# bcgsc/NanoSim

Measured on AMD Instinct MI355X. Metric: simulated reads/sec (genome mode, mean 8 kb), higher is better.
Workload: dtype u8

## Files before the change

### nanosim_amd/csrc/nanosim_amd.hip

```cpp
#include <hip/hip_runtime.h>
#include <hipcub/hipcub.hpp>
#include <stdio.h>
#include <stdlib.h>
#include <string.h>
#include <algorithm>
#include <chrono>
#include <atomic>
#include <condition_variable>
#include <functional>
#include <mutex>
#include <thread>
#include <type_traits>
#include <string>
#include <vector>

#include "ns_device.h"
#include "ns_materialise.h"
#include "ns_chain.h"
#include "ns_hp.h"
#include "ns_ir.h"
#include "ns_io.h"
#include "ns_pack.h"
#include "ns_cs_hist.h"
#include "ns_qual_hist.h"
// ... 965 lines not shown
    rd.rec_off = uni64(A.rec_off[r]);
    rd.piece_off = uni(rd.piece_off); rd.n_pieces = (uint16_t)uni(rd.n_pieces);
    rd.reversed = (uint8_t)uni(rd.reversed); rd.head = uni(rd.head); rd.tail = uni(rd.tail); rd.seq_len = uni(rd.seq_len);
    rd.attempts = uni(rd.attempts);
    key = read_key(A, r);
    key.r_lo = uni(key.r_lo); key.r_hi = uni(key.r_hi);
    ro.seq = A.records + rd.rec_off + uni(A.name_len[r]) + 2;
    ro.qual = fastq ? ro.seq + rd.seq_len + 3 : nullptr;
    ro.seq_len = rd.seq_len; ro.reversed = rd.reversed != 0; ro.uracil = A.prm.uracil != 0;
    return true;
}

#ifndef NS_MATQ_WAVES
#define NS_MATQ_WAVES 4
#endif
#ifndef NS_MATQ_MINW
#define NS_MATQ_MINW 6
#endif
__device__ __forceinline__ uint64_t hp_ev_slot(uint32_t hp_shift, uint32_t hp_pad, uint64_t pos, uint32_t piece) { return (pos >> hp_shift) + (uint64_t)hp_pad * piece; }
__device__ __forceinline__ uint64_t hp_ev_slot(const GenArgs &A, uint64_t pos, uint32_t piece) { return hp_ev_slot(A.hp_shift, A.hp_pad, pos, piece); }

#ifndef NS_TILE_CHUNKS_FINAL
#define NS_TILE_CHUNKS_FINAL 4u
#endif
#ifndef NS_MAT_WAVES_FINAL
#define NS_MAT_WAVES_FINAL 6
#endif
struct MatArgs { GenArgs A; SlowQueue sq; const uint32_t *order; uint32_t dbg; };
typedef const __attribute__((address_space(4))) MatArgs *MatArgsPtr;
__device__ __forceinline__ MatArgsPtr mat_args_now() {
    MatArgsPtr p = (MatArgsPtr)__builtin_amdgcn_kernarg_segment_ptr();
    asm volatile("" : "+s"(p));
    return p;
}
struct MatCold {
    uint32_t gp, pi;
    __device__ __forceinline__ void push(uint32_t lane, uint32_t m0, uint32_t m1) const {
        const uint32_t *order = mat_args_now()->order;
        const uint32_t r = order ? uni(order[blockIdx.x]) : blockIdx.x;
        const MatArgsPtr K = mat_args_now();
        SlowQueue sq; sq.items = K->sq.items; sq.count = K->sq.count; sq.cap = K->sq.cap;
        slow_queue_push(sq, lane, SlowTile{r, pi, m0, m1});
    }
    __device__ __forceinline__ uint64_t chrom_len() const {
        const MatArgsPtr K = mat_args_now();
        const ns_piece *pieces = K->A.pieces;
        const uint64_t *off = K->A.ref.chrom_off;
        const uint32_t chrom = uni(pieces[gp].chrom);
        return uni64(off[chrom + 1]) - uni64(off[chrom]);
    }
};

template <bool FASTQ, int MODE, uint32_t TC, bool URACIL>
__device__ __forceinline__ uint32_t materialise_pieces(const GenArgs &A, TileLds<TC> &T, const ReadOut &ro, const ns_key &key, const ns_read &rd,
                                                       uint64_t r, uint32_t q, uint32_t lane, uint32_t dbg) {
    constexpr bool CLSOUT = FASTQ && MODE != MAT_HP_SCRATCH;
    const uint32_t a = rd.attempts;
    uint32_t *cls = nullptr;
    if constexpr (CLSOUT) cls = A.cls + cls_word0(rd.rec_off, r, cls_per_read(A.prm));
    uint64_t q_in = MODE == MAT_HP_FINAL ? uni64(A.scr_off[r]) : 0;
    for (uint32_t pi = 0; pi < rd.n_pieces; ++pi) {
        PieceCtx pc;
        const uint32_t gp = rd.piece_off + pi;
        if constexpr (MODE == MAT_HP_FINAL) {
            const MatArgsPtr K = mat_args_now();
            const ns_piece *pieces = K->A.pieces;
            const uint32_t *hp_pord = K->A.hp_pord, *hp_nev = K->A.hp_nev, *hp_len = K->A.hp_len;
            const ns_piece p = pieces[gp];
            const uint64_t eo = hp_ev_slot(K->A.hp_shift, K->A.hp_pad, q_in, uni(hp_pord[r]) + pi);
            pc.kind = uni(p.kind);
            pc.ev = K->A.hp_ev + eo; pc.wd = K->A.hp_wd + eo; pc.n_ev = pc.kind ? 0u : uni(hp_nev[gp]);
            pc.ref_len = uni(p.out_len); pc.out_len = pc.kind ? pc.ref_len : uni(hp_len[gp]);
            pc.chrom_base = (uint64_t)((uintptr_t)K->A.scr - (uintptr_t)K->A.ref.bases) + q_in; pc.chrom_len = ~0ull; pc.pos = 0;
            pc.sid = pc.kind ? NS_GAP_SEG + (pi >> 1) : (pi >> 1);
            q_in += pc.ref_len;
        } else pc = load_piece_uniform(A.events, A.ref, A.pieces[gp], pi);
        uint32_t *const pcls = CLSOUT ? cls + (q >> 4) + 2u * pi : nullptr;
        if (ro.reversed) materialise_piece<FASTQ, MODE, TC, true, URACIL>(A.ref, T, PieceOut<true>(ro, q), key, a, pc, lane, dbg, MatCold{gp, pi}, pcls);
        else materialise_piece<FASTQ, MODE, TC, false, URACIL>(A.ref, T, PieceOut<false>(ro, q), key, a, pc, lane, dbg, MatCold{gp, pi}, pcls);
        q += pc.out_len;
    }
    return q;
}

template <bool FASTQ, int MODE, bool URACIL>
__global__ void __launch_bounds__(64, MODE == MAT_HP_FINAL ? NS_MAT_WAVES_FINAL : NS_MAT_WAVES)
k_materialise(MatArgs K) {
    static_assert(std::is_trivially_copyable<MatArgs>::value && offsetof(MatArgs, A) == 0, "MatArgs is read back from the kernel-argument segment as it was passed");
    constexpr uint32_t TC = MODE == MAT_HP_FINAL ? NS_TILE_CHUNKS_FINAL : NS_TILE_CHUNKS;
    __shared__ TileLds<TC> T;
    const GenArgs &A = K.A;
    const uint32_t lane = threadIdx.x;
    const uint64_t slot = blockIdx.x;
    if (slot >= A.prm.n_reads) return;
    const uint64_t r = K.order ? (uint64_t)uni(K.order[slot]) : slot;
    ns_read rd; ns_key key; ReadOut ro;
    if (!load_read_uniform(A, r, false, rd, key, ro)) return;
    tile_lds_init(T, lane);
    if constexpr (MODE == MAT_HP_SCRATCH) {
        static_assert(MODE != MAT_HP_SCRATCH || !URACIL, "the scratch pass of -k writes T");
        ro.seq = A.scr + uni64(A.scr_off[r]); ro.qual = nullptr; ro.reversed = false; ro.uracil = false;
        materialise_pieces<FASTQ, MODE, TC, false>(A, T, ro, key, rd, r, 0u, lane, K.dbg);
    } else {
        ro.uracil = URACIL;
#ifdef NS_ABLATE
        if (!(K.dbg & 8))
#endif
        emit_head_tail(ro, key, rd.attempts, rd.head, rd.tail, lane);
        const uint32_t q = materialise_pieces<FASTQ, MODE, TC, URACIL>(A, T, ro, key, rd, r, rd.head, lane, K.dbg);
        if (A.polya) {
            const uint32_t pl = uni(A.polya[r]);
            if (pl) emit_polya(ro, q, pl, lane);
        }
    }
}

template <bool HPF>
__global__ void __launch_bounds__(64 * NS_MATQ_WAVES, NS_MATQ_MINW) k_qualities(GenArgs A, const uint32_t *order) {
    __shared__ __align__(16) uint16_t qlut[NS_QLUT_SLOTS * 1024u];
    qual_lut_load(qlut, A.m, threadIdx.x, 64 * NS_MATQ_WAVES);
    __syncthreads();
    const uint32_t lane = threadIdx.x & 63u;
    const uint64_t slot = (uint64_t)blockIdx.x * NS_MATQ_WAVES + (threadIdx.x >> 6);
    if (slot >= A.prm.n_reads) return;
    const uint64_t r = order ? (uint64_t)uni(order[slot]) : slot;
    ns_read rd; ns_key key; ReadOut ro;
    if (!load_read_uniform(A, r, true, rd, key, ro)) return;
    const uint32_t a = rd.attempts;
    QualState Q; Q.lut = qlut;
    qualities_head_tail(A.m, Q, ro, key, a, rd.head, rd.tail, lane);
    const uint32_t *cls = A.cls + cls_word0(rd.rec_off, r, cls_per_read(A.prm));
    uint32_t q = rd.head;
    for (uint32_t pi = 0; pi < rd.n_pieces; ++pi) {
        const uint32_t gp = rd.piece_off + pi;
        const ns_piece p = A.pieces[gp];
        const uint32_t kind = uni(p.kind);
        const uint32_t out_len = (HPF && !kind) ? uni(A.hp_len[gp]) : uni(p.out_len);
        qualities_piece(A.m, Q, ro, key, a, kind ? NS_GAP_SEG + (pi >> 1) : (pi >> 1), kind, out_len, q, cls + (q >> 4) + 2u * pi, lane);
        q += out_len;
    }
    if (A.polya) {
        const uint32_t pl = uni(A.polya[r]);
        if (pl) emit_polya_quals(A.m, ro, key, a, q, pl, rd.head, rd.tail, lane);
    }
}

#define NS_DENSE_SEG 4096u
__global__ void __launch_bounds__(256) k_dense_plan(GenArgs A, uint32_t *cnt) {
    const uint64_t r = (uint64_t)blockIdx.x * blockDim.x + threadIdx.x;
    if (r > A.prm.n_reads) return;
    uint32_t c = 0;
    if (r < A.prm.n_reads) { const ns_read rd = A.reads[r]; c = rd.flags ? 0u : max(1u, (rd.seq_len + NS_DENSE_SEG - 1u) / NS_DENSE_SEG); }
    cnt[r] = c;
}
__global__ void __launch_bounds__(64) k_materialise_dense(GenArgs A, const uint32_t *__restrict__ seg_off) {
    __shared__ DenseLds S;
    const uint32_t lane = threadIdx.x;
    const uint32_t w = blockIdx.x, n = (uint32_t)A.prm.n_reads;
    if (w >= seg_off[n]) return;
    uint32_t lo = 0, hi = n;
    while (hi - lo > 1) { const uint32_t mid = (lo + hi) >> 1; if (seg_off[mid] <= w) lo = mid; else hi = mid; }
    const uint64_t r = uni(lo);
    const uint32_t seg = uni(w - seg_off[lo]);
    ns_read rd; ns_key key; ReadOut ro;
    if (!load_read_uniform(A, r, false, rd, key, ro)) return;
    const uint32_t a = rd.attempts;
    if (seg == 0) emit_head_tail(ro, key, a, rd.head, rd.tail, lane);
    uint32_t q = rd.head;
    for (uint32_t pi = 0; pi < rd.n_pieces; ++pi) {
        const PieceCtx pc = load_piece_uniform(A.events, A.ref, A.pieces[rd.piece_off + pi], pi);
        const uint64_t s_lo = (uint64_t)seg * NS_DENSE_SEG, s_hi = s_lo + NS_DENSE_SEG, p_lo = q - rd.head, p_hi = p_lo + pc.out_len;
        if (p_hi > s_lo && p_lo < s_hi) {
            const uint32_t m_lo = (uint32_t)(max(s_lo, p_lo) - p_lo), m_hi = (uint32_t)(min(s_hi, p_hi) - p_lo);
            if (A.dbg & 16384u) slow_piece_range(A.m, A.ref, ro, key, a, pc, q, m_lo, m_hi, lane);
            else dense_piece(A.m, A.ref, S, ro, key, a, pc, q, m_lo, m_hi, lane);
        }
        q += pc.out_len;
    }
}

template <bool FASTQ, bool SCRATCH>
__global__ void __launch_bounds__(64) k_materialise_slow(GenArgs A, SlowQueue sq) {
    const uint32_t lane = threadIdx.x;
    const uint32_t n = min(*sq.count, sq.cap);
    for (uint32_t i = blockIdx.x; i < n; i += gridDim.x) {
        const SlowTile t = sq.items[i];
        ns_read rd; ns_key key; ReadOut ro;
        if (!load_read_uniform(A, t.read, FASTQ && !SCRATCH, rd, key, ro)) continue;
        uint32_t q = SCRATCH ? 0u : rd.head;
        if constexpr (SCRATCH) { ro.seq = A.scr + A.scr_off[t.read]; ro.qual = nullptr; ro.reversed = false; ro.uracil = false; }
        for (uint32_t pi = 0; pi < t.piece; ++pi) q += A.pieces[rd.piece_off + pi].out_len;
        const PieceCtx pc = load_piece_uniform(A.events, A.ref, A.pieces[rd.piece_off + t.piece], t.piece);
        slow_piece_range<FASTQ && SCRATCH>(A.m, A.ref, ro, key, rd.attempts, pc, q, t.m0, t.m1, lane);
    }
}

template <bool FASTQ>
__global__ void __launch_bounds__(64) k_materialise_slow_hpf(GenArgs A, SlowQueue sq) {
    const uint32_t lane = threadIdx.x;
    const uint32_t n = min(*sq.count, sq.cap);
    for (uint32_t i = blockIdx.x; i < n; i += gridDim.x) {
        const SlowTile t = sq.items[i];
        ns_read rd; ns_key key; ReadOut ro;
        if (!load_read_uniform(A, t.read, FASTQ, rd, key, ro)) continue;
        uint32_t q = rd.head;
        uint64_t q_in = A.scr_off[t.read];
        for (uint32_t pi = 0; pi < t.piece; ++pi) {
            const uint32_t gp = rd.piece_off + pi;
            const ns_piece p = A.pieces[gp];
            q += p.kind ? p.out_len : A.hp_len[gp];
            q_in += p.out_len;
        }
        const uint32_t gp = rd.piece_off + t.piece;
        const ns_piece p = A.pieces[gp];
        const uint64_t eo = hp_ev_slot(A, q_in, A.hp_pord[t.read] + t.piece);
        const ns_event *ev = A.hp_ev + eo;
        const uint32_t *wd = A.hp_wd + eo;
        const uint32_t n_ev = p.kind ? 0u : A.hp_nev[gp], sid = p.kind ? NS_GAP_SEG + (t.piece >> 1) : (t.piece >> 1);
        const uint8_t *src = A.scr + q_in;
// ... 3059 lines not shown
```

### nanosim_amd/csrc/ns_device.h

```cpp
#pragma once
#include "ns_rng.h"
#include "../../include/nanosim_amd.h"

enum NsStat : uint32_t {
    NS_STAT_OVER,
    NS_STAT_BASES,
    NS_STAT_REF_BASES,
    NS_STAT_EVENTS,
    NS_STAT_MAX_READ,
    NS_STAT_HP_FAILED,
    NS_STAT_NEXT_N,
    NS_STAT_HP_OVER,
    NS_STAT_HP_RANGE,
    NS_STAT_COUNT
};
#define NS_RANGE_SHIFT 40
#define NS_OVER_MASK ((1ull << NS_RANGE_SHIFT) - 1)
#define NS_STATS_WAYS 64u
#define NS_STATS_BYTES ((NS_STAT_COUNT + NS_STAT_COUNT * NS_STATS_WAYS) * sizeof(unsigned long long))
__host__ __device__ inline unsigned long long *ns_stats_way(unsigned long long *stats, uint32_t way) { return stats + NS_STAT_COUNT + NS_STAT_COUNT * way; }

struct ChainTab {
    uint32_t n_words;
    uint32_t trans;
// ... 272 lines not shown
    for (int e = 0; e < 12; ++e) {
        const uint32_t i = (uint32_t)list[e].code & 31u;
        uint32_t k = 0;
        for (; list[e].mem[k]; ++k) {
            const char b = list[e].mem[k];
            p.slot[k] |= (uint64_t)(b == 'A' ? 0 : b == 'T' ? 1 : b == 'C' ? 2 : 3) << (2u * i);
        }
        p.cnt |= (uint64_t)(k - 1u) << (2u * i);
    }
    return p;
}
NS_DEV uint32_t iupac_members(uint32_t c, uint32_t &n) {
    constexpr IupacPack P = iupac_pack();
    const uint32_t sh = 2u * (c & 31u);
    const uint32_t code = (c >> 5) == 2u ? (uint32_t)(P.cnt >> sh) & 3u : 0u;
    n = code + (code != 0u);
    uint32_t mem = 0;
    for (uint32_t k = 0; k < 4u; ++k) mem |= ((0x47435441u >> (8u * ((uint32_t)(P.slot[k] >> sh) & 3u))) & 0xffu) << (8u * k);
    return code ? mem & (0xffffffffu >> (8u * (3u - code))) : 0u;
}
NS_DEV uint8_t normalise_base(uint32_t c) {
    c &= 0x7fu;
    if (c >= 'a' && c <= 'z') c -= 32;
    uint32_t n;
    if (is_acgt(c)) return (uint8_t)c;
    iupac_members(c, n);
    return (uint8_t)((n ? c : (uint32_t)'N') | 0x80u);
}
NS_DEV uint8_t resolve_base(uint32_t c, const ns_key &key, uint32_t seg, uint32_t attempt, uint32_t x) {
    if (!(c & 0x80u)) return (uint8_t)c;
    c &= 0x7fu;
    uint32_t n, mem = iupac_members(c, n);
    if (!n) return (uint8_t)c;
    u32x4 w = ns_draw(key, ST_IUPAC, seg, attempt, x >> 2, 0);
    uint32_t j = (uint32_t)(((uint64_t)ns_word(w, x & 3) * n) >> 32);
    return (uint8_t)(mem >> (8 * j));
}
NS_DEV uint32_t payload_word(const ns_key &key, uint32_t seg, uint32_t attempt, uint32_t j, uint32_t c) {
    if (c == 0) { u32x4 w = ns_draw(key, ST_SUB, seg, attempt, j >> 2, 0); return ns_word(w, j & 3); }
    u32x4 w = ns_draw(key, ST_INS, seg, attempt, j, c >> 2);
    return ns_word(w, c & 3);
}
NS_DEV uint8_t mis_from_digit(uint32_t cur, uint32_t dg) {
    int rc = base_rank(cur);
    uint32_t rk = dg + ((int)dg >= rc ? 1u : 0u);
    if (rc < 0) rk = dg;
    return bases_atcg(rk);
}
NS_DEV uint32_t next_digit3(uint32_t &frac) {
    uint64_t p = (uint64_t)frac * 3u;
    frac = (uint32_t)p;
    return (uint32_t)(p >> 32);
}
__device__ __forceinline__ uint8_t mis_letter(uint32_t cur, const ns_key &key, uint32_t seg, uint32_t attempt, uint32_t j, uint32_t i) {
    uint32_t frac = payload_word(key, seg, attempt, j, i >> 4), dg = 0;
    for (uint32_t t = 0; t <= (i & 15); ++t) dg = next_digit3(frac);
    return mis_from_digit(cur, dg);
}
__device__ __forceinline__ uint8_t ins_letter(const ns_key &key, uint32_t seg, uint32_t attempt, uint32_t j, uint32_t i) {
    return bases_atcg((payload_word(key, seg, attempt, j, i >> 4) >> (2 * (i & 15))) & 3u);
}
__device__ __forceinline__ uint8_t ht_letter(const ns_key &key, uint32_t stream, uint32_t attempt, uint32_t i) {
    u32x4 w = ns_draw(key, stream, 0, attempt, i >> 6, 0);
    return bases_atcg((ns_word(w, (i >> 4) & 3) >> (2 * (i & 15))) & 3u);
}
NS_DEV uint8_t qual_value_lut(const uint32_t *__restrict__ thr, const uint16_t *__restrict__ lut, uint32_t h) {
    const uint32_t e = lut[h >> 6];
    if (!(e & 0x8000u)) return (uint8_t)(((e & 0x7fffu) + (h & 63u)) >> 7);
    uint32_t q = (e >> 7) & 0x7fu;
    while (q < NS_QUAL_LEVELS - 1 && h >= thr[q]) ++q;
    return (uint8_t)q;
}
NS_DEV uint8_t qual_value(const uint32_t *__restrict__ thr, uint32_t h) {
    uint32_t lo = 0, hi = NS_QUAL_LEVELS - 1;
    while (lo < hi) {
        uint32_t mid = (lo + hi) >> 1;
        if (h >= thr[mid]) lo = mid + 1; else hi = mid;
    }
    return (uint8_t)lo;
}
__device__ __forceinline__ uint8_t qual_at(const DevModel &m, int cls, const ns_key &key, uint32_t stream, uint32_t seg,
                                           uint32_t attempt, uint32_t mpos) {
    u32x4 w = ns_draw(key, stream, seg, attempt, mpos >> 3, 0);
    uint32_t h = (ns_word(w, (mpos & 7) >> 1) >> (16 * (mpos & 1))) & 0xffffu;
    return qual_value(m.qual_thr + cls * NS_QUAL_LEVELS, h);
}

NS_DEV uint32_t dec_digits(uint32_t v) {
    return v < 10u ? 1u : v < 100u ? 2u : v < 1000u ? 3u : v < 10000u ? 4u : v < 100000u ? 5u : v < 1000000u ? 6u : v < 10000000u ? 7u :
           v < 100000000u ? 8u : v < 1000000000u ? 9u : 10u;
}
NS_DEV uint8_t *put_dec(uint8_t *p, uint32_t v) {
    const uint32_t n = dec_digits(v);
    for (uint32_t i = 0; i < n; ++i) { const uint32_t q = v / 10u; p[n - 1 - i] = (uint8_t)('0' + (v - 10u * q)); v = q; }
    return p + n;
}
template <class P>
NS_DEV P put_dec_p(P p, uint32_t v) {
    const uint32_t n = dec_digits(v);
    for (uint32_t i = 0; i < n; ++i) { const uint32_t q = v / 10u; p[n - 1 - i] = (uint8_t)('0' + (v - 10u * q)); v = q; }
    return p + n;
}
__device__ __forceinline__ uint32_t dec_digits(uint64_t v) {
    uint32_t n = 1;
    while (v >= 10) { v /= 10; ++n; }
    return n;
// ... 14 lines not shown
```

### nanosim_amd/csrc/ns_materialise.h

```cpp
#pragma once
#include "ns_device.h"

#ifndef NS_TILE_CHUNKS
#define NS_TILE_CHUNKS 2u
#endif
#define T_EV 64u
#define NS_CLS_MIS_BIT 0x08u
#define NS_CLS_INS_BIT 0x20u
#define NS_CLS_STRIP 0xd7d7d7d7u
#define NS_QLUT_SLOTS 5u
__device__ __forceinline__ uint32_t wave_incl_scan(uint32_t v) {
    v += (uint32_t)__builtin_amdgcn_update_dpp(0, (int)v, 0x111, 0xf, 0xf, true);
    v += (uint32_t)__builtin_amdgcn_update_dpp(0, (int)v, 0x112, 0xf, 0xf, true);
    v += (uint32_t)__builtin_amdgcn_update_dpp(0, (int)v, 0x114, 0xf, 0xf, true);
    v += (uint32_t)__builtin_amdgcn_update_dpp(0, (int)v, 0x118, 0xf, 0xf, true);
    v += (uint32_t)__builtin_amdgcn_update_dpp(0, (int)v, 0x142, 0xa, 0xf, false);
    v += (uint32_t)__builtin_amdgcn_update_dpp(0, (int)v, 0x143, 0xc, 0xf, false);
    return v;
}

__device__ __forceinline__ uint32_t wave_incl_max(uint32_t v) {
    v = max(v, (uint32_t)__builtin_amdgcn_update_dpp(0, (int)v, 0x111, 0xf, 0xf, false));
    v = max(v, (uint32_t)__builtin_amdgcn_update_dpp(0, (int)v, 0x112, 0xf, 0xf, false));
    v = max(v, (uint32_t)__builtin_amdgcn_update_dpp(0, (int)v, 0x114, 0xf, 0xf, false));
    v = max(v, (uint32_t)__builtin_amdgcn_update_dpp(0, (int)v, 0x118, 0xf, 0xf, false));
    v = max(v, (uint32_t)__builtin_amdgcn_update_dpp(0, (int)v, 0x142, 0xa, 0xf, false));
    v = max(v, (uint32_t)__builtin_amdgcn_update_dpp(0, (int)v, 0x143, 0xc, 0xf, false));
    return v;
}
__device__ __forceinline__ uint32_t dpp_wave_shl1(uint32_t lane63_value, uint32_t v) {
    return (uint32_t)__builtin_amdgcn_update_dpp((int)lane63_value, (int)v, 0x130, 0xf, 0xf, false);
}

__device__ __forceinline__ uint32_t uni(uint32_t v) { return (uint32_t)__builtin_amdgcn_readfirstlane((int)v); }
__device__ __forceinline__ uint64_t uni64(uint64_t v) { return (uint64_t)uni((uint32_t)v) | (uint64_t)uni((uint32_t)(v >> 32)) << 32; }

__device__ __forceinline__ uint32_t here(uint32_t v) { asm volatile("" : "+s"(v)); return v; }

struct ReadOut {
    uint8_t *seq;
    uint8_t *qual;
    uint32_t seq_len;
    bool reversed;
    bool uracil;
};
__device__ __forceinline__ uint64_t t_to_u8(uint64_t x) {
    const uint64_t t = x ^ 0x5454545454545454ull;
    const uint64_t z = ~(((t & 0x7f7f7f7f7f7f7f7full) + 0x7f7f7f7f7f7f7f7full) | t) & 0x8080808080808080ull;
    return x | (z >> 7);
}

typedef uint32_t ns_v4u_any __attribute__((ext_vector_type(4), aligned(1)));
__device__ __forceinline__ void store16(uint8_t *dst, uint32_t count, uint64_t lo, uint64_t hi) {
    if (count == 16) {
        ns_v4u_any x = {(uint32_t)lo, (uint32_t)(lo >> 32), (uint32_t)hi, (uint32_t)(hi >> 32)};
        __builtin_nontemporal_store(x, reinterpret_cast<ns_v4u_any *>(dst));
    } else {
        if (count & 8u) { __builtin_memcpy(dst, &lo, 8); dst += 8; lo = hi; }
// ... 233 lines not shown
    }
}

__device__ __forceinline__ void wave_sync() {
    __builtin_amdgcn_fence(__ATOMIC_ACQ_REL, "wavefront");
    __builtin_amdgcn_wave_barrier();
}

typedef __attribute__((address_space(3))) volatile uint8_t *LdsBytes;
typedef __attribute__((address_space(3))) volatile uint32_t *LdsWords;
__device__ __forceinline__ void lds_put_bytes(LdsBytes d, uint32_t x0, uint32_t x1, uint32_t x2, uint32_t x3, uint32_t cn) {
    const uint32_t head = min(cn, (0u - (uint32_t)(uintptr_t)d) & 3u);
    if (head > 0) d[0] = (uint8_t)x0;
    if (head > 1) d[1] = (uint8_t)(x0 >> 8);
    if (head > 2) d[2] = (uint8_t)(x0 >> 16);
    const uint32_t sh = 8u * head;
    const uint32_t y0 = __builtin_amdgcn_alignbit(x1, x0, sh), y1 = __builtin_amdgcn_alignbit(x2, x1, sh), y2 = __builtin_amdgcn_alignbit(x3, x2, sh), y3 = x3 >> sh;
    const uint32_t rem = cn - head;
    const LdsWords w = (LdsWords)(d + head);
    if (rem >= 4u) w[0] = y0;
    if (rem >= 8u) w[1] = y1;
    if (rem >= 12u) w[2] = y2;
    if (rem >= 16u) w[3] = y3;
    const uint32_t yt = rem >= 12u ? y3 : rem >= 8u ? y2 : rem >= 4u ? y1 : y0, tail = rem & 3u;
    const LdsBytes e = d + head + (rem & ~3u);
    if (tail > 0) e[0] = (uint8_t)yt;
    if (tail > 1) e[1] = (uint8_t)(yt >> 8);
    if (tail > 2) e[2] = (uint8_t)(yt >> 16);
}

NS_DEV uint32_t marked4(uint32_t w) { return (((w >> 7) & 0x01010101u) * 0x01020408u) >> 24; }
NS_DEV void resolve16(uint32_t &a0, uint32_t &a1, uint32_t &a2, uint32_t &a3, uint32_t among, uint32_t x0,
                      const ns_key &key, uint32_t sid, uint32_t a) {
    uint32_t mk = (marked4(a0) | marked4(a1) << 4 | marked4(a2) << 8 | marked4(a3) << 12) & among;
    while (mk) {
        const uint32_t b = (uint32_t)__builtin_ctz(mk), sh = 8u * (b & 3u);
        mk &= mk - 1u;
        uint32_t wk = b < 8 ? (b < 4 ? a0 : a1) : (b < 12 ? a2 : a3);
        const uint32_t r = resolve_base((wk >> sh) & 0xffu, key, sid, a, x0 + b);
        wk = (wk & ~(0xffu << sh)) | r << sh;
        if (b < 4) a0 = wk; else if (b < 8) a1 = wk; else if (b < 12) a2 = wk; else a3 = wk;
    }
}
NS_DEV void resolve4(uint32_t &w, uint32_t among, uint32_t x0, const ns_key &key, uint32_t sid, uint32_t a) {
    uint32_t mk = marked4(w) & among;
    while (mk) {
        const uint32_t b = (uint32_t)__builtin_ctz(mk), sh = 8u * b;
        mk &= mk - 1u;
        w = (w & ~(0xffu << sh)) | (uint32_t)resolve_base((w >> sh) & 0xffu, key, sid, a, x0 + b) << sh;
    }
}

#define NS_DENSE_TILE 1024u
struct __align__(16) DenseLds { uint8_t out[NS_DENSE_TILE + 64]; };

__device__ inline void dense_piece(const DevModel &m, const DevRef &ref, DenseLds &S, const ReadOut &ro, const ns_key &key, uint32_t a,
                                   const PieceCtx &pc, uint32_t pq, uint32_t m_lo, uint32_t m_hi, uint32_t lane) {
    if (m_lo & 15u) { slow_piece_range(m, ref, ro, key, a, pc, pq, m_lo, m_hi, lane); return; }
    const uint32_t n_items = pc.n_ev + 1u;
    const uint8_t *seg0 = ref.bases + pc.chrom_base + pc.pos;
    const uint64_t lin = pc.chrom_len - pc.pos;
    uint32_t jb = 0;
    if (m_lo) jb = uni(events_up_to(pc.ev, pc.n_ev, m_lo));
    for (uint32_t M0 = m_lo; M0 < m_hi; M0 += NS_DENSE_TILE) {
        const uint32_t M1 = min(M0 + NS_DENSE_TILE, m_hi);
        uint32_t seen = 0;
        for (uint32_t jj0 = jb;; jj0 += 64) {
            const uint32_t jj = jj0 + lane;
            const bool valid = jj < n_items;
            uint32_t os = 0, pl = 0, ty = 3, rp = 0, pos = 0, nxt = pc.out_len;
            if (valid) {
                if (jj) {
                    const ns_event e = pc.ev[jj - 1];
                    const uint32_t len = ns_ev_len(e.info);
                    ty = ns_ev_type(e.info); os = ev_out_start(e); pos = e.pos;
                    pl = ev_letters(ty, len); rp = ev_resume(e.pos, ty, len);
                }
                if (jj < pc.n_ev) nxt = ev_out_start(pc.ev[jj]);
            }
            const uint32_t lo = max(os, M0), hi = min(nxt, M1);
            const bool act = valid && lo < hi;
            const uint32_t n_let = act ? min(pl, hi - os) : 0u;
            const uint32_t c_lo = max(lo, os + pl);
            const uint32_t cn = act && c_lo < hi ? hi - c_lo : 0u;
            const uint32_t x0 = rp + (c_lo - os - pl);
            const bool fast_l = n_let && os >= M0 && (ty == NS_INS || (uint64_t)pos + n_let <= lin);
            const bool fast_c = cn && cn <= 16u && (uint64_t)x0 + 16u <= lin;
            uint4 f = make_uint4(0, 0, 0, 0);
            if (fast_c) __builtin_memcpy(&f, seg0 + x0, 16);
            if ((f.x | f.y | f.z | f.w) & 0x80808080u) resolve16(f.x, f.y, f.z, f.w, 0xffffu >> (16u - cn), x0, key, pc.sid, a);
            {
                uint32_t nl_max = fast_l ? n_let : 0u;
                nl_max = max(nl_max, (uint32_t)__builtin_amdgcn_update_dpp(0, (int)nl_max, 0x111, 0xf, 0xf, false));
                nl_max = max(nl_max, (uint32_t)__builtin_amdgcn_update_dpp(0, (int)nl_max, 0x112, 0xf, 0xf, false));
                nl_max = max(nl_max, (uint32_t)__builtin_amdgcn_update_dpp(0, (int)nl_max, 0x114, 0xf, 0xf, false));
                nl_max = max(nl_max, (uint32_t)__builtin_amdgcn_update_dpp(0, (int)nl_max, 0x118, 0xf, 0xf, false));
                const uint32_t m01 = max((uint32_t)__builtin_amdgcn_readlane((int)nl_max, 15), (uint32_t)__builtin_amdgcn_readlane((int)nl_max, 31));
                const uint32_t m23 = max((uint32_t)__builtin_amdgcn_readlane((int)nl_max, 47), (uint32_t)__builtin_amdgcn_readlane((int)nl_max, 63));
                const uint32_t groups = (max(m01, m23) + 3u) >> 2;
                uint32_t frac = 0;
                const uint32_t o_base = os - M0;
                for (uint32_t g = 0; g < groups; ++g) {
                    const uint32_t i0 = 4u * g;
                    const bool on = fast_l && i0 < n_let;
                    if (!(g & 3u) && on) frac = payload_word(key, pc.sid, a, jj - 1u, g >> 2);
                    uint32_t cur4 = 0x41414141u;
                    if (on && ty != NS_INS) {
                        __builtin_memcpy(&cur4, seg0 + pos + i0, 4);
                        if (cur4 & 0x80808080u) resolve4(cur4, 0xfu >> (4u - min(4u, n_let - i0)), pos + i0, key, pc.sid, a);
                    }
                    const uint32_t ins4 = ins_letters4(frac, g & 3u);
                    uint32_t f3 = frac;
                    const uint32_t d0 = next_digit3(f3), d1 = next_digit3(f3), d2 = next_digit3(f3), d3 = next_digit3(f3);
                    const uint32_t d4 = d0 | d1 << 8 | d2 << 16 | d3 << 24;
                    const uint32_t vv = (cur4 >> 1) & 0x03030303u;
                    const uint32_t rank4 = (vv & 0x01010101u) << 1 | ((vv >> 1) & 0x01010101u);
                    const uint32_t ge = ((d4 | 0x80808080u) - rank4) & 0x80808080u;
                    const uint32_t mis4 = __builtin_amdgcn_perm(0u, 0x47435441u, d4 + (ge >> 7));
                    const bool is_ins = ty == NS_INS;
                    if (!is_ins) frac = f3;
                    const uint32_t letters = is_ins ? ins4 : mis4;
                    const uint32_t cnt = on ? n_let - i0 : 0u, dump = NS_DENSE_TILE + lane, o = o_base + i0;
                    S.out[cnt > 0 ? o : dump] = (uint8_t)letters; S.out[cnt > 1 ? o + 1 : dump] = (uint8_t)(letters >> 8);
                    S.out[cnt > 2 ? o + 2 : dump] = (uint8_t)(letters >> 16); S.out[cnt > 3 ? o + 3 : dump] = (uint8_t)(letters >> 24);
                }
            }
            if (fast_c) lds_put_bytes((LdsBytes)&S.out[c_lo - M0], f.x, f.y, f.z, f.w, cn);
            if (act && ((n_let && !fast_l) || (cn && !fast_c))) {
                if (!fast_l) {
                    uint32_t word = 0;
                    for (uint32_t i = 0; i < n_let; ++i) {
                        if (!(i & 15u)) word = payload_word(key, pc.sid, a, jj - 1u, i >> 4);
                        uint32_t b;
                        if (ty == NS_INS) b = bases_atcg((word >> (2u * (i & 15u))) & 3u);
                        else {
                            const uint32_t x = pos + i;
                            b = mis_from_digit(resolve_base(ref_base_at(ref, pc, x), key, pc.sid, a, x), next_digit3(word));
                        }
                        if (os + i >= lo) S.out[os + i - M0] = (uint8_t)b;
                    }
                }
                if (cn && !fast_c) {
                    for (uint32_t i = 0; i < cn; ++i) {
                        const uint32_t x = x0 + i;
                        S.out[c_lo + i - M0] = resolve_base(ref_base_at(ref, pc, x), key, pc.sid, a, x);
                    }
                }
            }
            seen += (uint32_t)__popcll(__ballot(valid && os <= M1));
            if (__ballot(valid && os >= M1) || jj0 + 64u >= n_items) break;
        }
        jb = jb + seen - 1u;
        wave_sync();
        const uint32_t m0 = M0 + 16u * lane;
        if (m0 < M1) {
            const uint32_t count = min(16u, M1 - m0);
            const uint4 v = *reinterpret_cast<const uint4 *>(&S.out[16u * lane]);
            store_chunk(ro, pq + m0, count, (uint64_t)v.x | (uint64_t)v.y << 32, (uint64_t)v.z | (uint64_t)v.w << 32, 0, 0);
        }
        wave_sync();
    }
}


struct SlowTile { uint32_t read, piece, m0, m1; };
struct SlowQueue { SlowTile *items; uint32_t *count; uint32_t cap; };
__device__ __forceinline__ void slow_queue_push(const SlowQueue &sq, uint32_t lane, const SlowTile &t) {
// ... 39 lines not shown
        const uint32_t E = __builtin_bit_cast(uint32_t, e2);
        flags |= E;
        const ns_v2u16 s2 = (__builtin_bit_cast(ns_v2u16, E) + __builtin_bit_cast(ns_v2u16, d & 0x003f003fu)) >> (uint16_t)7;
        Q2[k] = __builtin_bit_cast(uint32_t, s2);
    }
    if (__ballot((flags & 0x80008000u) != 0)) {
#pragma unroll
        for (uint32_t k = 0; k < 8; ++k) {
            const uint32_t c0 = (cs[k >> 1] >> (16 * (k & 1) + 3)) & 7u, c1 = (cs[k >> 1] >> (16 * (k & 1) + 11)) & 7u;
            const uint32_t q0 = qual_value(m.qual_thr + min(c0, (uint32_t)NS_Q_COUNT - 1u) * NS_QUAL_LEVELS, D[k] & 0xffffu);
            const uint32_t q1 = qual_value(m.qual_thr + min(c1, (uint32_t)NS_Q_COUNT - 1u) * NS_QUAL_LEVELS, D[k] >> 16);
            Q2[k] = q0 | q1 << 16;
        }
    }
    const uint32_t b0 = __builtin_amdgcn_perm(Q2[1], Q2[0], 0x06040200u), b1 = __builtin_amdgcn_perm(Q2[3], Q2[2], 0x06040200u);
    const uint32_t b2 = __builtin_amdgcn_perm(Q2[5], Q2[4], 0x06040200u), b3 = __builtin_amdgcn_perm(Q2[7], Q2[6], 0x06040200u);
    qlo = (uint64_t)b0 | (uint64_t)b1 << 32; qhi = (uint64_t)b2 | (uint64_t)b3 << 32;
}
__device__ __forceinline__ uint32_t cls_pack16(uint32_t r0, uint32_t r1, uint32_t r2, uint32_t r3) {
    auto field = [](uint32_t r) {
        const uint32_t t = and_or(r >> 4, 0x02020202u, (r >> 3) & 0x01010101u);
        return t * 0x01041040u;
    };
    const uint32_t p0 = field(r0), p1 = field(r1), p2 = field(r2), p3 = field(r3);
    return __builtin_amdgcn_perm(p1, p0, 0x0c0c0703u) | __builtin_amdgcn_perm(p3, p2, 0x07030c0cu);
}
__device__ __forceinline__ uint32_t cls_unpack4(uint32_t w, uint32_t k) {
    const uint32_t e = (w >> (8u * k)) & 0xffu;
    uint32_t t = e << 3;
    t |= e << 9; t |= e << 15; t |= e << 21;
    return t & 0x18181818u;
}
__device__ __forceinline__ uint64_t cls_word0(uint64_t rec_off, uint64_t r, uint32_t per_read) { return (rec_off >> 4) + r * per_read; }
__device__ __forceinline__ uint32_t cls_per_read(const ns_params &prm) { return prm.chimeric ? 2u * (2u * NS_MAX_SEG - 1u) : 2u; }

__device__ __forceinline__ void qual_lut_load(uint16_t *lds, const DevModel &m, uint32_t tid, uint32_t nthreads) {
    const uint4 *src = reinterpret_cast<const uint4 *>(m.qual_lut);
    uint4 *dst = reinterpret_cast<uint4 *>(lds);
    for (uint32_t i = tid; i < NS_QLUT_SLOTS * 128u; i += nthreads) dst[i] = src[i];
}

__device__ __forceinline__ void lds_or32(uint8_t *p, uint32_t v) {
    __hip_atomic_fetch_or(reinterpret_cast<unsigned int *>(p), v, __ATOMIC_RELAXED, __HIP_MEMORY_SCOPE_WAVEFRONT);
}
__device__ __forceinline__ void lds_or64(uint8_t *p, uint64_t v) {
    __hip_atomic_fetch_or(reinterpret_cast<unsigned long long *>(p), (unsigned long long)v, __ATOMIC_RELAXED, __HIP_MEMORY_SCOPE_WAVEFRONT);
}

template <int MODE>
__device__ __forceinline__ uint32_t event_word(const PieceCtx &pc, const ns_key &key, uint32_t a, uint32_t j) {
    if constexpr (MODE == MAT_HP_FINAL) return pc.wd[j];
    else { const u32x4 w = ns_draw(key, ST_SUB, pc.sid, a, j >> 2, 0); return ns_word(w, j & 3u); }
}
template <uint32_t TC>
struct __align__(16) TileLds {
    static constexpr uint32_t T_OUT_ = 1024u * TC;
    uint32_t mlut[17][4];
    uint2 ent[T_EV + 1];
    uint32_t eos[T_EV + 1];
    uint32_t hist[64 * TC];
    __align__(16) uint8_t out[1024u * TC + 16 + 64];
};
template <uint32_t TC>
__device__ __forceinline__ void tile_lds_init(TileLds<TC> &T, uint32_t lane) {
    for (uint32_t c = lane * 16; c < 1024u * TC + 16 + 64; c += 64 * 16) *reinterpret_cast<uint4 *>(&T.out[c]) = make_uint4(0, 0, 0, 0);
    if (lane < 17) {
#pragma unroll
        for (uint32_t k = 0; k < 4; ++k)
            T.mlut[lane][k] = lane <= 4 * k ? 0xffffffffu : lane >= 4 * k + 4 ? 0u : 0xffffffffu << (8 * (lane - 4 * k));
    }
}
#ifdef NS_ABLATE
#define NS_DBG(bit) (dbg & (bit))
#else
#define NS_DBG(bit) false
#endif
__device__ __forceinline__ uint32_t and_andn(uint32_t a, uint32_t b, uint32_t c) { return __builtin_amdgcn_bitop3_b32(a, b, c, 0x40); }
template <bool FASTQ, int MODE, uint32_t TC, bool REV, bool URACIL, typename Cold>
__device__ inline void materialise_piece(const DevRef &ref, TileLds<TC> &T, const PieceOut<REV> out, const ns_key &key,
                                         uint32_t a, const PieceCtx &pc, uint32_t lane, uint32_t dbg, const Cold &cold,
                                         uint32_t *__restrict__ cls) {
    constexpr bool CLSOUT = FASTQ && MODE != MAT_HP_SCRATCH;
    constexpr bool HPF = MODE == MAT_HP_FINAL;
    constexpr uint32_t T_OUT_ = 1024u * TC;
    uint32_t jb = 0;
    uint32_t L0_out = 0, L0_rp = 0, L0_pt = 3u << 12, L0_wd = 0, L0_j = 0;
    const uint8_t *seg0 = ref.bases + pc.chrom_base + pc.pos;
    const uint32_t wrap_at = (!HPF && pc.pos + pc.ref_len > pc.chrom_len) ? (uint32_t)(pc.chrom_len - pc.pos) : 0xffffffffu;
    const uint32_t fast_pl = wrap_at != 0xffffffffu ? 0u : 8u;
    auto base_at = [&](uint32_t x) -> uint32_t { const uint8_t *s = seg0; if (!HPF && x >= wrap_at) s -= cold.chrom_len(); return s[x]; };
    const uint32_t phi = out.phi();
    ns_event e_pre; e_pre.pos = 0; e_pre.info = 0; uint32_t w_pre = 0;
    if (lane < pc.n_ev) e_pre = pc.ev[lane];
    auto cached_word = [&](uint32_t j0) -> uint32_t { if (NS_DBG(64u)) return 0u; const uint32_t j = j0 + lane; return event_word<MODE>(pc, key, a, j < pc.n_ev ? j : 0u); };
    w_pre = cached_word(0u);
    uint32_t cls_carry = 0;
    for (uint32_t M0 = 0; M0 < pc.out_len;) {
        const uint32_t A0 = M0 - ((M0 - phi) & 15u);
        uint32_t M1 = min(A0 + T_OUT_, pc.out_len);
        const ns_event e = e_pre;
        const uint32_t e_wd = w_pre;
        const bool valid = jb + lane < pc.n_ev;
        const uint32_t os = ev_out_start(e), len = ns_ev_len(e.info), ty = ns_ev_type(e.info);
        const uint32_t e_pt = ev_letters(ty, len) | ty << 12, e_rp = ev_resume(e.pos, ty, len);
        if (jb + 63 < pc.n_ev) {
            const uint32_t os63 = (uint32_t)__builtin_amdgcn_readlane((int)os, 63);
            if (os63 < M1) {
                const uint32_t cut = A0 + ((os63 - A0) & ~15u);
                M1 = (int32_t)(cut - M0) > 0 ? cut : os63;
            }
        }
        const bool take = valid && os < M1;
        const uint32_t cnt = (uint32_t)__popcll(__ballot(take));
        if (M1 <= M0) {
            cls_carry = 0;
            M1 = min(M0 + T_OUT_, pc.out_len);
            uint32_t j2 = jb;
            while (j2 < pc.n_ev && ev_out_start(pc.ev[j2]) < M1) ++j2;
            cold.push(lane, M0, M1);
            if (j2 > jb) {
                const ns_event le = pc.ev[j2 - 1];
                const uint32_t ll = ns_ev_len(le.info), lt = ns_ev_type(le.info);
                L0_out = uni(ev_out_start(le)); L0_pt = uni(ev_letters(lt, ll) | lt << 12); L0_rp = uni(ev_resume(le.pos, lt, ll));
                L0_wd = uni(event_word<MODE>(pc, key, a, j2 - 1)); L0_j = uni(j2 - 1);
            }
            jb = uni(j2); M0 = M1;
            e_pre.pos = 0; e_pre.info = 0; w_pre = 0;
            if (jb + lane < pc.n_ev) e_pre = pc.ev[jb + lane];
            w_pre = cached_word(jb);
            continue;
        }
        const uint32_t nc = (M1 - A0 + 15u) >> 4;
        const uint32_t ekey = take ? (os <= M0 ? 0u : (os - A0 + 15u) >> 4) : 0xffffffffu;
        const uint32_t s1 = os + (e_pt & 0xfffu), y1 = e_rp - s1;
        {
            const uint32_t s0 = L0_out + (L0_pt & 0xfffu);
            T.ent[0] = make_uint2(s0, L0_rp - s0);
            if (take) T.ent[1 + lane] = make_uint2(s1, y1);
            T.eos[lane] = take ? os : 0xffffffffu;
        }
#pragma unroll
        for (uint32_t t = 0; t < TC; ++t) T.hist[64 * t + lane] = 0;
        const uint32_t jb_next = jb + cnt;
        e_pre.pos = 0; e_pre.info = 0; w_pre = 0;
        if (M1 < pc.out_len && jb_next + lane < pc.n_ev) e_pre = pc.ev[jb_next + lane];
        if (M1 < pc.out_len) w_pre = cached_word(jb_next);
        wave_sync();
        const uint32_t os_next = dpp_wave_shl1(0xffffffffu, take ? os : 0xffffffffu);
        {
            const uint32_t c_next = dpp_wave_shl1(0xffffffffu, ekey);
            if (ekey < 64 * TC && ekey != c_next) T.hist[ekey] = lane + 1u;
        }
        uint32_t osl = L0_out, ptl = L0_pt, rpl = L0_rp, wdl = L0_wd, jl = L0_j;
        if (cnt) {
            osl = (uint32_t)__builtin_amdgcn_readlane((int)os, (int)(cnt - 1));
            ptl = (uint32_t)__builtin_amdgcn_readlane((int)e_pt, (int)(cnt - 1));
            rpl = (uint32_t)__builtin_amdgcn_readlane((int)e_rp, (int)(cnt - 1));
            wdl = (uint32_t)__builtin_amdgcn_readlane((int)e_wd, (int)(cnt - 1));
            jl = jb + cnt - 1;
        }
        const uint8_t *tb = seg0 - 32;
        bool fast = true;
        if (!HPF && here(wrap_at) != 0xffffffffu) {
            const uint32_t pl0 = L0_pt & 0xfffu, ty0 = L0_pt >> 12, d0 = M0 - L0_out;
            const uint32_t x0 = (d0 < pl0 && ty0 == NS_INS) ? L0_rp : L0_rp + d0 - pl0;
            const uint32_t pll = ptl & 0xfffu, dl = M1 - osl;
            uint32_t x1 = dl <= pll ? rpl : rpl + (dl - pll);
            if (x1 < x0) x1 = x0;
            if (x0 >= wrap_at) tb -= cold.chrom_len();
            else if (x1 > wrap_at) fast = false;
        }
        if (!fast) {
            cls_carry = 0;
            cold.push(lane, M0, M1);
            L0_out = osl; L0_rp = rpl; L0_pt = ptl; L0_wd = wdl; L0_j = jl;
            jb = jb_next; M0 = M1;
            wave_sync();
            continue;
        }
        wave_sync();
        uint4 f[TC]; uint32_t fi[TC], fy[TC];
        {
            uint32_t scan_base = 0;
#pragma unroll
            for (uint32_t t = 0; t < TC; ++t) {
                const uint32_t ci = 64 * t + lane;
                const uint32_t incl = max(scan_base, wave_incl_max(T.hist[ci]));
                scan_base = (uint32_t)__builtin_amdgcn_readlane((int)incl, 63);
                f[t] = make_uint4(0, 0, 0, 0); fi[t] = 16u | 16u << 8; fy[t] = 0;
                if (ci < nc && !NS_DBG(1u) && !NS_DBG(256u)) {
                    const uint32_t cs = A0 + 16u * ci, p = ci == 0 ? M0 : cs;
                    const uint2 E = T.ent[incl];
                    const uint32_t nx = T.eos[incl];
                    const uint32_t st = max(p, E.x), en = min(nx, min(cs + 16u, M1));
                    if ((int32_t)(en - st) > 0) {
                        fi[t] = (st - cs) | (en - cs) << 8; fy[t] = E.y;
                        __builtin_memcpy(&f[t], tb + (E.y + cs + 32u), 16);
                    }
                }
            }
        }
        uint4 fe = make_uint4(0, 0, 0, 0); uint32_t ei0 = 16, ei1 = 16, eoc = 0;
        if (take && !NS_DBG(1u) && !NS_DBG(128u)) {
            const uint32_t c = (s1 - A0) >> 4, ecs = A0 + 16u * c;
            const uint32_t en = min(os_next, min(ecs + 16u, M1));
            if ((int32_t)(en - s1) > 0 && ekey > c) {
                eoc = 16u * c; ei0 = s1 - ecs; ei1 = en - ecs;
                __builtin_memcpy(&fe, tb + (y1 + ecs + 32u), 16);
            }
        }
        if (!NS_DBG(2u)) {
            const bool cont = lane == 63 && L0_out + (L0_pt & 0xfffu) > M0;
            const uint32_t b_os = cont ? L0_out : os, b_pt = cont ? L0_pt : e_pt, b_rp = cont ? L0_rp : e_rp;
            const uint32_t b_j = cont ? L0_j : jb + lane;
            uint32_t frac = cont ? L0_wd : e_wd;
            const uint32_t b_pl = b_pt & 0xfffu, b_ty = b_pt >> 12;
            const bool on = (take || cont) && b_pl;
            const uint32_t xs = b_rp - b_pl;
            const bool mis = b_ty == NS_MIS;
            bool fast_l = on && b_pl <= fast_pl && b_os >= M0 && b_os + b_pl <= M1;
            uint2 cur8 = make_uint2(0x41414141u, 0x41414141u);
            if (fast_l && mis) __builtin_memcpy(&cur8, seg0 + xs, 8);
            const uint64_t keep = b_pl >= 8u ? ~0ull : ~(~0ull << (8u * b_pl));
            if constexpr (!HPF) fast_l = fast_l && !(((uint64_t)cur8.x | (uint64_t)cur8.y << 32) & keep & 0x8080808080808080ull);
            if (fast_l) {
                uint32_t f3 = frac, L2[2];
#pragma unroll
                for (uint32_t g = 0; g < 2; ++g) {
                    const uint32_t cur4 = g ? cur8.y : cur8.x;
                    const uint32_t ins4 = ins_letters4(frac, g);
                    const uint32_t d0 = next_digit3(f3), d1 = next_digit3(f3), d2 = next_digit3(f3), d3 = next_digit3(f3);
                    const uint32_t d4 = d0 | d1 << 8 | d2 << 16 | d3 << 24;
                    const uint32_t vv = (cur4 >> 1) & 0x03030303u;
                    const uint32_t rank4 = (vv & 0x01010101u) << 1 | ((vv >> 1) & 0x01010101u);
                    const uint32_t ge = ((d4 | 0x80808080u) - rank4) & 0x80808080u;
                    const uint32_t mis4 = __builtin_amdgcn_perm(0u, 0x47435441u, d4 + (ge >> 7));
                    uint32_t letters = mis ? mis4 : ins4;
                    if constexpr (FASTQ) {
                        uint32_t cls4 = mis ? 0x01010101u * NS_CLS_MIS_BIT : 0x01010101u * NS_CLS_INS_BIT;
                        if constexpr (HPF) {
                            if (mis) cls4 = (frac & 1u) ? NS_CLS_MIS_BIT : (cur4 & (NS_CLS_MIS_BIT | NS_CLS_INS_BIT));
                            else if (g == 0 && (frac >> 31)) cls4 = (cls4 & ~0xffu) | NS_CLS_MIS_BIT;
                        }
                        letters |= cls4;
                    }
                    L2[g] = letters;
                }
                const uint64_t v = ((uint64_t)L2[0] | (uint64_t)L2[1] << 32) & keep;
                const uint32_t o = b_os - A0, sh = 8u * (o & 3u);
                const uint64_t lo64 = v << sh;
                const uint32_t top = (uint32_t)(((v >> 32) << sh) >> 32);
                uint8_t *w = &T.out[o & ~3u];
                lds_or32(w, (uint32_t)lo64); lds_or32(w + 4, (uint32_t)(lo64 >> 32)); lds_or32(w + 8, top);
            }
            if (on && !fast_l) {
                const uint32_t i_lo = b_os < M0 ? M0 - b_os : 0u;
                const uint32_t i_hi = min(b_pl, M1 - b_os);
                const uint32_t word0 = frac;
                for (uint32_t i = 0; i < i_hi; ++i) {
                    if (i && !(i & 15)) frac = payload_word(key, pc.sid, a, b_j, i >> 4);
                    uint32_t b;
                    if (b_ty == NS_INS) {
                        b = bases_atcg((frac >> (2 * (i & 15))) & 3u);
                        if constexpr (FASTQ) b |= (HPF && i == 0 && (word0 >> 31)) ? NS_CLS_MIS_BIT : NS_CLS_INS_BIT;
                    } else {
                        const uint32_t x = xs + i;
                        const uint32_t src = base_at(x);
                        if constexpr (HPF) {
                            b = mis_from_digit(src & ~(NS_CLS_MIS_BIT | NS_CLS_INS_BIT), next_digit3(frac));
                            if constexpr (FASTQ) b |= (word0 & 1u) ? NS_CLS_MIS_BIT : (src & (NS_CLS_MIS_BIT | NS_CLS_INS_BIT));
                        } else {
                            b = mis_from_digit(resolve_base(src, key, pc.sid, a, x), next_digit3(frac));
                            if constexpr (FASTQ) b |= NS_CLS_MIS_BIT;
                        }
                    }
                    if (i >= i_lo) T.out[b_os + i - A0] = (uint8_t)b;
                }
            }
        }
        if (cnt && ei0 < 16u && !NS_DBG(32u)) {
            const uint4 m0 = *reinterpret_cast<const uint4 *>(&T.mlut[ei0][0]), m1 = *reinterpret_cast<const uint4 *>(&T.mlut[ei1][0]);
            uint32_t a0 = and_andn(fe.x, m0.x, m1.x), a1 = and_andn(fe.y, m0.y, m1.y), a2 = and_andn(fe.z, m0.z, m1.z), a3 = and_andn(fe.w, m0.w, m1.w);
            if constexpr (!HPF) {
                if ((a0 | a1 | a2 | a3) & 0x80808080u) resolve16(a0, a1, a2, a3, 0xffffu, A0 + eoc + y1, key, pc.sid, a);
            }
// ... 89 lines not shown
```

Baseline: 136.9 million.

## Batch per-event random words into LDS window and table-lookup base-3 digits

Replaces four sequential base-3 digit extractions with one multiply by 81 and a lookup into an LDS table of packed digit quadruples. Per-event substitution words are now drawn in bulk, four per lane, into a 256-entry LDS window that is refilled only when the event range moves past it. This applies to both the tiled and dense materialise kernels. It removes repeated RNG draws and several multiplies per group, at the cost of more LDS per block, extra wave syncs, and table initialisation at kernel start.

```diff
diff --git a/nanosim_amd/csrc/nanosim_amd.hip b/nanosim_amd/csrc/nanosim_amd.hip
--- a/nanosim_amd/csrc/nanosim_amd.hip
+++ b/nanosim_amd/csrc/nanosim_amd.hip
@@ -1041,7 +1041,7 @@
 };
 
 template <bool FASTQ, int MODE, uint32_t TC, bool URACIL>
-__device__ __forceinline__ uint32_t materialise_pieces(const GenArgs &A, TileLds<TC> &T, const ReadOut &ro, const ns_key &key, const ns_read &rd,
+__device__ __forceinline__ uint32_t materialise_pieces(const GenArgs &A, TileLds<TC, MODE != MAT_HP_FINAL> &T, const ReadOut &ro, const ns_key &key, const ns_read &rd,
                                                        uint64_t r, uint32_t q, uint32_t lane, uint32_t dbg) {
     constexpr bool CLSOUT = FASTQ && MODE != MAT_HP_SCRATCH;
     const uint32_t a = rd.attempts;
@@ -1077,7 +1077,7 @@
 k_materialise(MatArgs K) {
     static_assert(std::is_trivially_copyable<MatArgs>::value && offsetof(MatArgs, A) == 0, "MatArgs is read back from the kernel-argument segment as it was passed");
     constexpr uint32_t TC = MODE == MAT_HP_FINAL ? NS_TILE_CHUNKS_FINAL : NS_TILE_CHUNKS;
-    __shared__ TileLds<TC> T;
+    __shared__ TileLds<TC, MODE != MAT_HP_FINAL> T;
     const GenArgs &A = K.A;
     const uint32_t lane = threadIdx.x;
     const uint64_t slot = blockIdx.x;
@@ -1154,6 +1154,8 @@
     ns_read rd; ns_key key; ReadOut ro;
     if (!load_read_uniform(A, r, false, rd, key, ro)) return;
     const uint32_t a = rd.attempts;
+    dense_lds_init(S, lane);
+    wave_sync();
     if (seg == 0) emit_head_tail(ro, key, a, rd.head, rd.tail, lane);
     uint32_t q = rd.head;
     for (uint32_t pi = 0; pi < rd.n_pieces; ++pi) {
diff --git a/nanosim_amd/csrc/ns_device.h b/nanosim_amd/csrc/ns_device.h
--- a/nanosim_amd/csrc/ns_device.h
+++ b/nanosim_amd/csrc/ns_device.h
@@ -348,6 +348,21 @@
     frac = (uint32_t)p;
     return (uint32_t)(p >> 32);
 }
+#define NS_DIGITS4_N 81u
+NS_DEV constexpr uint32_t digits4_pack(uint32_t hi) {
+    return hi / 27u | (hi / 9u % 3u) << 8 | (hi / 3u % 3u) << 16 | (hi % 3u) << 24;
+}
+NS_DEV uint32_t digits4(uint32_t &frac) {
+    const uint64_t p = (uint64_t)frac * NS_DIGITS4_N;
+    frac = (uint32_t)p;
+    return digits4_pack((uint32_t)(p >> 32));
+}
+template <typename Tab>
+NS_DEV uint32_t digits4(uint32_t &frac, const Tab &tab) {
+    const uint64_t p = (uint64_t)frac * NS_DIGITS4_N;
+    frac = (uint32_t)p;
+    return tab[(uint32_t)(p >> 32)];
+}
 __device__ __forceinline__ uint8_t mis_letter(uint32_t cur, const ns_key &key, uint32_t seg, uint32_t attempt, uint32_t j, uint32_t i) {
     uint32_t frac = payload_word(key, seg, attempt, j, i >> 4), dg = 0;
     for (uint32_t t = 0; t <= (i & 15); ++t) dg = next_digit3(frac);
diff --git a/nanosim_amd/csrc/ns_materialise.h b/nanosim_amd/csrc/ns_materialise.h
--- a/nanosim_amd/csrc/ns_materialise.h
+++ b/nanosim_amd/csrc/ns_materialise.h
@@ -4,6 +4,7 @@
 #ifndef NS_TILE_CHUNKS
 #define NS_TILE_CHUNKS 2u
 #endif
+#define NS_WD_WIN 256u
 #define T_EV 64u
 #define NS_CLS_MIS_BIT 0x08u
 #define NS_CLS_INS_BIT 0x20u
@@ -343,7 +344,14 @@
 }
 
 #define NS_DENSE_TILE 1024u
-struct __align__(16) DenseLds { uint8_t out[NS_DENSE_TILE + 64]; };
+struct __align__(16) DenseLds {
+    uint8_t out[NS_DENSE_TILE + 64];
+    uint32_t dig[NS_DIGITS4_N];
+    __align__(16) uint32_t wd[4u + NS_WD_WIN];
+};
+__device__ __forceinline__ void dense_lds_init(DenseLds &S, uint32_t lane) {
+    for (uint32_t h = lane; h < NS_DIGITS4_N; h += 64) S.dig[h] = digits4_pack(h);
+}
 
 __device__ inline void dense_piece(const DevModel &m, const DevRef &ref, DenseLds &S, const ReadOut &ro, const ns_key &key, uint32_t a,
                                    const PieceCtx &pc, uint32_t pq, uint32_t m_lo, uint32_t m_hi, uint32_t lane) {
@@ -353,12 +361,21 @@
     const uint64_t lin = pc.chrom_len - pc.pos;
     uint32_t jb = 0;
     if (m_lo) jb = uni(events_up_to(pc.ev, pc.n_ev, m_lo));
+    uint32_t E0 = 0xffffffffu;
     for (uint32_t M0 = m_lo; M0 < m_hi; M0 += NS_DENSE_TILE) {
         const uint32_t M1 = min(M0 + NS_DENSE_TILE, m_hi);
         uint32_t seen = 0;
         for (uint32_t jj0 = jb;; jj0 += 64) {
             const uint32_t jj = jj0 + lane;
             const bool valid = jj < n_items;
+            const uint32_t e_lo = max(jj0, 1u) - 1u;
+            if (!(E0 <= e_lo && jj0 + 63u <= E0 + NS_WD_WIN)) {
+                E0 = e_lo & ~3u;
+                const u32x4 w = ns_draw(key, ST_SUB, pc.sid, a, (E0 >> 2) + lane, 0);
+                *reinterpret_cast<uint4 *>(&S.wd[4u + 4u * lane]) = make_uint4(w.x, w.y, w.z, w.w);
+                wave_sync();
+            }
+            const uint32_t word0 = S.wd[3u + jj0 - E0 + lane];
             uint32_t os = 0, pl = 0, ty = 3, rp = 0, pos = 0, nxt = pc.out_len;
             if (valid) {
                 if (jj) {
@@ -394,7 +411,7 @@
                 for (uint32_t g = 0; g < groups; ++g) {
                     const uint32_t i0 = 4u * g;
                     const bool on = fast_l && i0 < n_let;
-                    if (!(g & 3u) && on) frac = payload_word(key, pc.sid, a, jj - 1u, g >> 2);
+                    if (!(g & 3u) && on) frac = g ? payload_word(key, pc.sid, a, jj - 1u, g >> 2) : word0;
                     uint32_t cur4 = 0x41414141u;
                     if (on && ty != NS_INS) {
                         __builtin_memcpy(&cur4, seg0 + pos + i0, 4);
@@ -402,8 +419,7 @@
                     }
                     const uint32_t ins4 = ins_letters4(frac, g & 3u);
                     uint32_t f3 = frac;
-                    const uint32_t d0 = next_digit3(f3), d1 = next_digit3(f3), d2 = next_digit3(f3), d3 = next_digit3(f3);
-                    const uint32_t d4 = d0 | d1 << 8 | d2 << 16 | d3 << 24;
+                    const uint32_t d4 = digits4(f3, S.dig);
                     const uint32_t vv = (cur4 >> 1) & 0x03030303u;
                     const uint32_t rank4 = (vv & 0x01010101u) << 1 | ((vv >> 1) & 0x01010101u);
                     const uint32_t ge = ((d4 | 0x80808080u) - rank4) & 0x80808080u;
@@ -549,7 +565,7 @@
     if constexpr (MODE == MAT_HP_FINAL) return pc.wd[j];
     else { const u32x4 w = ns_draw(key, ST_SUB, pc.sid, a, j >> 2, 0); return ns_word(w, j & 3u); }
 }
-template <uint32_t TC>
+template <uint32_t TC, bool WORDS>
 struct __align__(16) TileLds {
     static constexpr uint32_t T_OUT_ = 1024u * TC;
     uint32_t mlut[17][4];
@@ -557,9 +573,12 @@
     uint32_t eos[T_EV + 1];
     uint32_t hist[64 * TC];
     __align__(16) uint8_t out[1024u * TC + 16 + 64];
+    __align__(16) uint32_t wd[WORDS ? NS_WD_WIN : 4u];
+    uint32_t dig[NS_DIGITS4_N];
 };
-template <uint32_t TC>
-__device__ __forceinline__ void tile_lds_init(TileLds<TC> &T, uint32_t lane) {
+template <uint32_t TC, bool WORDS>
+__device__ __forceinline__ void tile_lds_init(TileLds<TC, WORDS> &T, uint32_t lane) {
+    for (uint32_t h = lane; h < NS_DIGITS4_N; h += 64) T.dig[h] = digits4_pack(h);
     for (uint32_t c = lane * 16; c < 1024u * TC + 16 + 64; c += 64 * 16) *reinterpret_cast<uint4 *>(&T.out[c]) = make_uint4(0, 0, 0, 0);
     if (lane < 17) {
 #pragma unroll
@@ -574,7 +593,7 @@
 #endif
 __device__ __forceinline__ uint32_t and_andn(uint32_t a, uint32_t b, uint32_t c) { return __builtin_amdgcn_bitop3_b32(a, b, c, 0x40); }
 template <bool FASTQ, int MODE, uint32_t TC, bool REV, bool URACIL, typename Cold>
-__device__ inline void materialise_piece(const DevRef &ref, TileLds<TC> &T, const PieceOut<REV> out, const ns_key &key,
+__device__ inline void materialise_piece(const DevRef &ref, TileLds<TC, MODE != MAT_HP_FINAL> &T, const PieceOut<REV> out, const ns_key &key,
                                          uint32_t a, const PieceCtx &pc, uint32_t lane, uint32_t dbg, const Cold &cold,
                                          uint32_t *__restrict__ cls) {
     constexpr bool CLSOUT = FASTQ && MODE != MAT_HP_SCRATCH;
@@ -589,8 +608,26 @@
     const uint32_t phi = out.phi();
     ns_event e_pre; e_pre.pos = 0; e_pre.info = 0; uint32_t w_pre = 0;
     if (lane < pc.n_ev) e_pre = pc.ev[lane];
-    auto cached_word = [&](uint32_t j0) -> uint32_t { if (NS_DBG(64u)) return 0u; const uint32_t j = j0 + lane; return event_word<MODE>(pc, key, a, j < pc.n_ev ? j : 0u); };
-    w_pre = cached_word(0u);
+    uint32_t J0 = 0;
+    auto words_cover = [&](uint32_t j0, bool first) {
+        if constexpr (!HPF) {
+            if (first || j0 + 64u > J0 + NS_WD_WIN) {
+                J0 = first ? 0u : j0 & ~3u;
+                asm volatile("" : "+s"(J0));
+                if (!NS_DBG(64u)) {
+                    const u32x4 w = ns_draw(key, ST_SUB, pc.sid, a, (J0 >> 2) + lane, 0);
+                    *reinterpret_cast<uint4 *>(&T.wd[4u * lane]) = make_uint4(w.x, w.y, w.z, w.w);
+                }
+            }
+        }
+    };
+    auto words_at = [&](uint32_t j0) -> uint32_t {
+        if constexpr (HPF) { const uint32_t j = j0 + lane; return event_word<MODE>(pc, key, a, j < pc.n_ev ? j : 0u); }
+        else return T.wd[j0 - J0 + lane];
+    };
+    words_cover(0u, true);
+    if constexpr (!HPF) wave_sync();
+    w_pre = words_at(0u);
     uint32_t cls_carry = 0;
     for (uint32_t M0 = 0; M0 < pc.out_len;) {
         const uint32_t A0 = M0 - ((M0 - phi) & 15u);
@@ -624,7 +661,9 @@
             jb = uni(j2); M0 = M1;
             e_pre.pos = 0; e_pre.info = 0; w_pre = 0;
             if (jb + lane < pc.n_ev) e_pre = pc.ev[jb + lane];
-            w_pre = cached_word(jb);
+            words_cover(jb, false);
+            if constexpr (!HPF) wave_sync();
+            w_pre = words_at(jb);
             continue;
         }
         const uint32_t nc = (M1 - A0 + 15u) >> 4;
@@ -641,8 +680,9 @@
         const uint32_t jb_next = jb + cnt;
         e_pre.pos = 0; e_pre.info = 0; w_pre = 0;
         if (M1 < pc.out_len && jb_next + lane < pc.n_ev) e_pre = pc.ev[jb_next + lane];
-        if (M1 < pc.out_len) w_pre = cached_word(jb_next);
+        if (M1 < pc.out_len) { if constexpr (HPF) w_pre = words_at(jb_next); else words_cover(jb_next, false); }
         wave_sync();
+        if constexpr (!HPF) { if (M1 < pc.out_len) w_pre = words_at(jb_next); }
         const uint32_t os_next = dpp_wave_shl1(0xffffffffu, take ? os : 0xffffffffu);
         {
             const uint32_t c_next = dpp_wave_shl1(0xffffffffu, ekey);
@@ -726,8 +766,7 @@
                 for (uint32_t g = 0; g < 2; ++g) {
                     const uint32_t cur4 = g ? cur8.y : cur8.x;
                     const uint32_t ins4 = ins_letters4(frac, g);
-                    const uint32_t d0 = next_digit3(f3), d1 = next_digit3(f3), d2 = next_digit3(f3), d3 = next_digit3(f3);
-                    const uint32_t d4 = d0 | d1 << 8 | d2 << 16 | d3 << 24;
+                    const uint32_t d4 = digits4(f3, T.dig);
                     const uint32_t vv = (cur4 >> 1) & 0x03030303u;
                     const uint32_t rank4 = (vv & 0x01010101u) << 1 | ((vv >> 1) & 0x01010101u);
                     const uint32_t ge = ((d4 | 0x80808080u) - rank4) & 0x80808080u;
```

Result: no change. 138.3 million (median of 6 runs) (+1.0%).
